# alexmillerdb/two_tower_recommender_model

Hardware: AMD Instinct MI355X
Metric: training pairs/sec at batch 8192 (per GPU) (higher is better)
Workload: dtype fp32; 1 GPU; northstar: 100M items x 50M users, emb_dim 128, towers [128, 64], single-hot uniform ids; global_batch=8192, per_gpu_batch=8192, emb_dim=128, tower_dtype=bf16 (MFMA, fp32 acc), parallelism=single-gpu hipgraph

## Files before the change

two_tower_recommender_model_amd/csrc/tower_rows.hip:

```cpp
#include "tower_common.h"

namespace tt {


constexpr int RK_THREADS = 320;
__device__ __forceinline__ int rk_perm(int mt, int rho) {
  return 32 * (mt >> 1) + 8 * (rho >> 2) + 4 * (mt & 1) + (rho & 3);
}
__device__ __forceinline__ bf16x8 rk_afwd(const char* img, int mt, int s, int rho, int q) {
  return *reinterpret_cast<const bf16x8*>(img + rk_off(rk_perm(mt, rho), 32 * s + 8 * q));
}
__device__ __forceinline__ bf16x8 rk_abwd(const char* img, int mt, int s, int lane) {
  const int q = lane >> 4, qq = (lane >> 2) & 3, p = lane & 3;
  const int row = 32 * s + 8 * q + qq;
  const int col = 32 * (mt >> 1) + 8 * p + 4 * (mt & 1);
  const bf16x4 lo = __builtin_amdgcn_ds_read_tr16_b64_v4bf16((lds_bf16x4*)(img + rk_off(row, col)));
  const bf16x4 hi = __builtin_amdgcn_ds_read_tr16_b64_v4bf16((lds_bf16x4*)(img + rk_off(row + 4, col)));
  return __builtin_shufflevector(lo, hi, 0, 1, 2, 3, 4, 5, 6, 7);
}
__device__ __forceinline__ bf16x8 rk_pack(const f32x4& a, const f32x4& b) {
  bf16x8 v;
#pragma unroll
  for (int j = 0; j < 4; ++j) {
    v[j] = (__bf16)a[j];
    v[4 + j] = (__bf16)b[j];
  }
  return v;
}
template <int MT, int S, bool BWD>
__device__ __forceinline__ void rk_gemm(f32x4 (&acc)[8], const char* img, const bf16x8 (&b)[4], int lane) {
  const int n = lane & 15, q = lane >> 4;
  bf16x8 fa[2][MT];
#pragma unroll
  for (int mt = 0; mt < MT; ++mt) {
    acc[mt] = (f32x4)(0.f);
    fa[0][mt] = BWD ? rk_abwd(img, mt, 0, lane) : rk_afwd(img, mt, 0, n, q);
  }
#pragma unroll
  for (int s = 0; s < S; ++s) {
    if (s + 1 < S) {
#pragma unroll
      for (int mt = 0; mt < MT; ++mt)
        fa[(s + 1) & 1][mt] = BWD ? rk_abwd(img, mt, s + 1, lane) : rk_afwd(img, mt, s + 1, n, q);
    }
    __builtin_amdgcn_sched_barrier(0);
#pragma unroll
    for (int mt = 0; mt < MT; ++mt)
      acc[mt] = __builtin_amdgcn_mfma_f32_16x16x32_bf16(fa[s & 1][mt], b[s], acc[mt], 0, 0, 0);
    __builtin_amdgcn_sched_barrier(0);
  }
}
template <int X>
__device__ __forceinline__ float rk_xor(float v) {
  if constexpr (X == 1) return dpp_f<0xB1>(v);
  if constexpr (X == 2) return dpp_f<0x4E>(v);
  if constexpr (X == 4) return dpp_f<0x1B>(dpp_f<0x141>(v));
  return dpp_f<0x128>(v);
}
template <int X, int H>
__device__ __forceinline__ void rk_halve(float* v, int n) {
  const bool up = (n & X) != 0;
#pragma unroll
  for (int i = 0; i < H; ++i) {
    const float keep = up ? v[H + i] : v[i], send = up ? v[i] : v[H + i];
    v[i] = keep + rk_xor<X>(send);
  }
}
template <int NV>
__device__ __forceinline__ void rk_colsum(float (&v)[NV], int n) {
  static_assert(NV == 32 || NV == 16, "column sum of 32 or 16 values per lane");
  rk_halve<8, NV / 2>(v, n);
  rk_halve<4, NV / 4>(v, n);
  rk_halve<2, NV / 8>(v, n);
  rk_halve<1, NV / 16>(v, n);
}
template <int NS>
__device__ __forceinline__ void rk_strip(const bf16x8 (&v)[4], __bf16* row, int q) {
#pragma unroll
  for (int s = 0; s < NS; ++s) *reinterpret_cast<bf16x8*>(row + 32 * s + 8 * q) = v[s];
}

__device__ __forceinline__ char* px_row(const tt_peer_direct_t& x, int64_t row, int64_t row_bytes) {
  char* base = reinterpret_cast<char*>(x.row0[0]);
  int64_t f0 = 0;
#pragma unroll
  for (int q = 1; q < TT_PEER_MAXW; ++q) {
    if (q < x.W && row >= x.first_row[q]) {
      base = reinterpret_cast<char*>(x.row0[q]);
      f0 = x.first_row[q];
    }
  }
  return base + (row - f0) * row_bytes;
}
__device__ __forceinline__ bool px_copy_unit(const tt_peer_direct_t& x, int64_t u, const uint4*& src, uint4*& dst) {
  int64_t pre = 0;
  bool hit = false;
#pragma unroll
  for (int q = 0; q < TT_PEER_MAXW; ++q) {
    const int64_t n = q < x.W ? x.copy_len[q] >> 4 : 0;
    if (!hit && u >= pre && u < pre + n) {
      src = reinterpret_cast<const uint4*>(x.copy_src[q]) + (u - pre);
      dst = reinterpret_cast<uint4*>(x.copy_dst[q]) + (u - pre);
      hit = true;
    }
    pre += n;
  }
  return hit;
}
__device__ __forceinline__ int64_t px_copy_units(const tt_peer_direct_t& x) {
  int64_t n = 0;
#pragma unroll
  for (int q = 0; q < TT_PEER_MAXW; ++q) n += q < x.W ? x.copy_len[q] >> 4 : 0;
  return n;
}

struct RkRaw {
  uint32_t lo, hi;
};
__device__ __forceinline__ RkRaw rk_raw(const void* p, bool wide, int64_t i) {
  RkRaw r;
  if (wide) {
    const uint2 v = reinterpret_cast<const uint2*>(p)[i];
    r.lo = v.x;
    r.hi = v.y;
  } else {
    r.lo = reinterpret_cast<const uint32_t*>(p)[i];
    r.hi = 0u;
  }
  return r;
}
__device__ __forceinline__ int64_t rk_id(RkRaw r, bool wide) {
  return wide ? (int64_t)(((uint64_t)r.hi << 32) | r.lo) : (int64_t)(int32_t)r.lo;
}
__device__ __forceinline__ float rk_label(RkRaw r, int dt) {
  if (dt == TT_I32) return (float)(int32_t)r.lo;
  if (dt == TT_I64) return (float)(int64_t)(((uint64_t)r.hi << 32) | r.lo);
  return __uint_as_float(r.lo);
}
template <int N, typename T>
__device__ __forceinline__ void rk_pin(T (&p)[N]) {
  static_assert(N == 2 || N == 4 || N == 8, "2, 4 or 8 values");
  if constexpr (N == 8)
    asm volatile("" : "+v"(p[0]), "+v"(p[1]), "+v"(p[2]), "+v"(p[3]), "+v"(p[4]), "+v"(p[5]), "+v"(p[6]), "+v"(p[7]));
  else if constexpr (N == 4)
    asm volatile("" : "+v"(p[0]), "+v"(p[1]), "+v"(p[2]), "+v"(p[3]));
  else
    asm volatile("" : "+v"(p[0]), "+v"(p[1]));
}
#if TT_EXPERIMENTS
#define RK_STAMP(k) \
  do { if (a.stamps && lane == 0) a.stamps[8192 + ((int64_t)blockIdx.x * 16 + (k)) * 9 + wid] = (int64_t)__builtin_amdgcn_s_memrealtime(); } while (0)
#define RK_STAMP2(k) \
  do { if (a.stamps && lane == 0) a.stamps[8192 + ((int64_t)blockIdx.x * 16 + (k)) * 9 + 4 + wid] = (int64_t)__builtin_amdgcn_s_memrealtime(); } while (0)
#define RK_STAMP_IMG(k) \
  do { if (a.stamps && lane == 0) a.stamps[8192 + ((int64_t)blockIdx.x * 16 + (k)) * 9 + 8] = (int64_t)__builtin_amdgcn_s_memrealtime(); } while (0)
#else
#define RK_STAMP(k) do { } while (0)
#define RK_STAMP2(k) do { } while (0)
#define RK_STAMP_IMG(k) do { } while (0)
#endif

template <bool UPD, bool IDX, int IN, bool POOL = false>
__device__ __forceinline__ void tower_rows_body(const TowerArgs& a) {
  static_assert(IN == 128 || IN == 64, "row-owned T1: inputs of 128 or 64");
  static_assert(!POOL || (!UPD && !IDX), "pooled input: the plain T1 only");
  constexpr int NI = IN / 32;
  constexpr int MTI = IN / 16;
  __shared__ __attribute__((aligned(16))) char wimg[RK_IMG];
  __shared__ __attribute__((aligned(16))) float xo[2][2][16 * 64];
  __shared__ float bsum[2][RK_W0 + RK_W1];
  __shared__ float lrow[TR];
  __shared__ __attribute__((aligned(16))) float xr[4][16 * IN];
  const int lane = threadIdx.x & 63, wid = __builtin_amdgcn_readfirstlane(threadIdx.x >> 6);
  typedef __attribute__((address_space(3))) void lds_void;
  typedef __attribute__((address_space(1))) void glb_void;
  if (wid == 4) {
    RK_STAMP_IMG(0);
    if (!TDBG(16)) {
#pragma unroll
      for (int k = 0; k < RK_IMG / 1024; ++k)
        __builtin_amdgcn_global_load_lds((glb_void*)(a.wimg + k * 1024 + lane * 16), (lds_void*)(wimg + k * 1024), 16, 0, 0);
    }
    RK_STAMP_IMG(1);
    __builtin_amdgcn_s_waitcnt(0x0F70);
    RK_STAMP_IMG(2);
    __syncthreads();
    RK_STAMP_IMG(3);
    __syncthreads();
    __syncthreads();
    return;
  }
  const int t = wid >> 1, h = wid & 1, q = lane >> 4, n = lane & 15;
  const RkCommon& C = a.rk.c;
  const RkTower& T = a.rk.tw[t];
  const int64_t B = C.B;
  const void* const labels = C.labels;
  const int label_dtype = C.label_dtype, gid_dtype = C.gid_dtype;
  const void* const idcol = T.idcol;
  const void* const tab0 = T.tab;
  const int64_t gmod = T.gmod;
  const float* const b0p = T.b0;
  const float* const b1p = T.b1;
  const int32_t* const claim = T.claim;
  const int32_t* const pos_out = T.pos_out;
  const int64_t pstride = T.rstride;
  const int nwg = C.nwg;
  if (UPD) asm volatile("" ::"s"(nwg), "s"(B), "s"(labels), "s"(label_dtype), "s"(gid_dtype), "s"(idcol), "s"(tab0), "s"(gmod), "s"(b0p), "s"(b1p), "s"(claim));
  else if (IDX) asm volatile("" ::"s"(nwg), "s"(B), "s"(labels), "s"(label_dtype), "s"(idcol), "s"(tab0), "s"(b0p), "s"(b1p), "s"(pos_out));
  else if (POOL) asm volatile("" ::"s"(nwg), "s"(B), "s"(labels), "s"(label_dtype), "s"(tab0), "s"(b0p), "s"(b1p), "s"(pstride));
  else asm volatile("" ::"s"(nwg), "s"(B), "s"(labels), "s"(label_dtype), "s"(gid_dtype), "s"(idcol), "s"(tab0), "s"(gmod), "s"(b0p), "s"(b1p));
  const int tile = xcd_remap((int)blockIdx.x, nwg);
  const int64_t m0 = (int64_t)tile * TR, m = m0 + 16 * h + n;
  const bool live = m < B;
  RK_STAMP(0);
  const bool wide = gid_dtype == TT_I64;
  const int64_t mc = live ? m : 0;
  RkRaw id_raw{0u, 0u}, pout_raw{0u, 0u};
  if (IDX) {
    id_raw.lo = (uint32_t) reinterpret_cast<const int32_t*>(idcol)[mc];
    pout_raw.lo = pos_out ? (uint32_t)pos_out[mc] : id_raw.lo;
  } else if (!POOL) {
    id_raw = rk_raw(idcol, wide, mc);
  }
  int32_t cl = -1;
  if (UPD) cl = claim[mc];
  const RkRaw lab_raw = rk_raw(labels, label_dtype == TT_I64, mc);
  f32x4 b0v[8], b1v[4];
  auto load_biases = [&]() {
#pragma unroll
    for (int mt = 0; mt < 8; ++mt) b0v[mt] = *reinterpret_cast<const f32x4*>(b0p + 32 * (mt >> 1) + 8 * q + 4 * (mt & 1));
#pragma unroll
    for (int mt = 0; mt < 4; ++mt) b1v[mt] = *reinterpret_cast<const f32x4*>(b1p + 32 * (mt >> 1) + 8 * q + 4 * (mt & 1));
  };
  load_biases();
  __builtin_amdgcn_sched_barrier(0);
  uint4 cpv = make_uint4(0u, 0u, 0u, 0u);
  uint4* cpd = nullptr;
  int64_t cp_per = 0, cp_end = 0;
  if constexpr (IDX) {
    if (a.xd.W) {
      const int64_t tot = px_copy_units(a.xd);
      cp_per = (tot + gridDim.x - 1) / gridDim.x;
      cp_end = min(tot, ((int64_t)blockIdx.x + 1) * cp_per);
      const int64_t u = (int64_t)blockIdx.x * cp_per + threadIdx.x;
      const uint4* cps;
      if (u < cp_end && px_copy_unit(a.xd, u, cps, cpd)) cpv = *cps;
      else cpd = nullptr;
    }
  }
  int64_t r;
  if (POOL) {
    r = live ? m : -1;
  } else if (IDX) {
    r = live ? (int64_t)(int32_t)id_raw.lo : -1;
  } else {
    const int64_t id = live ? rk_id(id_raw, wide) : 0;
    r = id != 0 ? py_mod64(id, gmod) : -1;
  }
  const float* tab = reinterpret_cast<const float*>(tab0);
  const int64_t rstride = POOL ? pstride : IN;
  RK_STAMP2(4);
  __builtin_amdgcn_sched_barrier(0);
  float* xw = xr[wid];
  constexpr int CPR = IDX ? IN / 8 : IN / 4;
  constexpr int RPI = 64 / CPR;
  constexpr int NDMA = 16 / RPI;
  if (IDX) {
    const int rr0 = lane / CPR, pc = lane % CPR;
    const char* src0 = reinterpret_cast<const char*>(tab0);
    const char* src[NDMA];
    int64_t rid[NDMA];
#pragma unroll
    for (int i = 0; i < NDMA; ++i) rid[i] = __shfl((long long)r, RPI * i + rr0, 64);
    rk_pin<NDMA>(rid);
#pragma unroll
    for (int i = 0; i < NDMA; ++i) {
      const int row = RPI * i + rr0;
      src[i] = src0 + (rid[i] >= 0 ? rid[i] : 0) * (IN * 2) + 16 * (pc ^ (row & (CPR - 1)));
    }
    rk_pin<NDMA>(src);
#pragma unroll
    for (int i = 0; i < NDMA; ++i)
      __builtin_amdgcn_global_load_lds((glb_void*)src[i], (lds_void*)(reinterpret_cast<char*>(xw) + i * 1024), 16, 0, 0);
  } else {
    const int rr0 = lane / CPR, pc = lane % CPR;
    const float* src[NDMA];
    int64_t rid[NDMA];
#pragma unroll
    for (int i = 0; i < NDMA; ++i) rid[i] = __shfl((long long)r, RPI * i + rr0, 64);
    rk_pin<NDMA>(rid);
#pragma unroll
    for (int i = 0; i < NDMA; ++i) {
      const int row = RPI * i + rr0;
      src[i] = tab + (rid[i] >= 0 ? rid[i] : 0) * rstride + 4 * (pc ^ row);
    }
    rk_pin<NDMA>(src);
#pragma unroll
    for (int i = 0; i < NDMA; ++i)
      if (!TDBG(32))
        __builtin_amdgcn_global_load_lds((glb_void*)src[i], (lds_void*)(xw + i * 256), 16, 0, 0);
  }
  __builtin_amdgcn_sched_barrier(0);
  DdPend pend;
  pend.key = DD_EMPTY;
  const int32_t li = (int32_t)(t * B + m);
  if (!UPD && a.dd_on && q == 0 && live) {
    const uint64_t key = r >= 0 ? (((uint64_t)(t ? a.dd_table[1] : a.dd_table[0]) << DD_TABLE_SHIFT) | (uint64_t)r)
                                : DD_EMPTY;
    dd_insert_begin(a.dd, key, li, pend);
  }
  RK_STAMP(1);
  const int in_max = C.in_max;
  const float grad_scale = C.grad_scale, fB = C.fB;
  DSlot* const slots = C.slots;
  __bf16* const xt_t = T.xt;
  __bf16* const act_t = T.act0;
  const float* const us_t = T.us;
  __builtin_amdgcn_sched_barrier(0);
  __builtin_amdgcn_s_waitcnt(0x0F70);
  if (UPD) asm volatile("" ::"s"(in_max), "s"(grad_scale), "s"(fB), "s"(slots), "s"(xt_t), "s"(act_t), "s"(us_t));
  else asm volatile("" ::"s"(in_max), "s"(grad_scale), "s"(fB), "s"(xt_t), "s"(act_t));
  RK_STAMP(2);
  __syncthreads();
  RK_STAMP(3);
  f32x4 xv[8];
  bf16x8 xb[4];
  if (IDX) {
#pragma unroll
    for (int s2 = 0; s2 < NI; ++s2) {
      const bf16x8 v = *reinterpret_cast<const bf16x8*>(reinterpret_cast<const char*>(xw) + n * (IN * 2) +
                                                         16 * ((4 * s2 + q) ^ (n & (CPR - 1))));
      xb[s2] = r >= 0 ? v : (bf16x8)(__bf16)0.f;
    }
  } else {
#pragma unroll
    for (int mt = 0; mt < MTI; ++mt) {
      const int c = 8 * (mt >> 1) + 2 * q + (mt & 1);
      const f32x4 v = *reinterpret_cast<const f32x4*>(xw + n * IN + 4 * (c ^ n));
      xv[mt] = r >= 0 ? v : (f32x4)(0.f);
    }
#pragma unroll
    for (int s2 = 0; s2 < NI; ++s2) xb[s2] = rk_pack(xv[2 * s2], xv[2 * s2 + 1]);
  }
  uint32_t word = 0u;
  float s_old = 0.f;
  if (UPD) {
    if (blockIdx.x == 0 && threadIdx.x == 0) {
      int32_t* const ctr = C.ctr;
      const int32_t nh = ctr[0];
      ctr[2] = nh;
      ctr[0] = 0;
    }
    word = reinterpret_cast<const uint32_t*>(&slots[cl >= 0 ? cl : 0].word)[0];
    s_old = us_t[r >= 0 ? r : 0];
  }
  __builtin_amdgcn_sched_barrier(0);
  const char* img0 = wimg + t * RK_IMG_T;
  const char* img1 = img0 + RK_W0 * 256;
  f32x4 acc[8];
  if (!TDBG(512)) rk_strip<NI>(xb, xt_t + m * in_max, q);
  rk_gemm<8, NI, false>(acc, img0, xb, lane);
  RK_STAMP(4);
  bf16x8 hb[4];
#pragma unroll
  for (int s = 0; s < 4; ++s) {
    f32x4 u0, u1;
#pragma unroll
    for (int j = 0; j < 4; ++j) {
      u0[j] = fmaxf(acc[2 * s][j] + b0v[2 * s][j], 0.f);
      u1[j] = fmaxf(acc[2 * s + 1][j] + b0v[2 * s + 1][j], 0.f);
    }
    hb[s] = rk_pack(u0, u1);
  }
  if (!TDBG(256)) rk_strip<4>(hb, act_t + m * MAXW, q);
  f32x4 uo[4];
  rk_gemm<4, 4, false>(acc, img1, hb, lane);
#pragma unroll
  for (int mt = 0; mt < 4; ++mt) uo[mt] = acc[mt];
#pragma unroll
  for (int mt = 0; mt < 4; ++mt) {
#pragma unroll
    for (int j = 0; j < 4; ++j) uo[mt][j] = fmaxf(uo[mt][j] + b1v[mt][j], 0.f);
    const int c = 8 * (mt >> 1) + 2 * q + (mt & 1);
    *reinterpret_cast<f32x4*>(&xo[t][h][n * 64 + ((c ^ n) << 2)]) = uo[mt];
  }
  RK_STAMP(5);
  RK_STAMP(6);
  __syncthreads();
  RK_STAMP(7);
  f32x4 vo[4];
#pragma unroll
  for (int mt = 0; mt < 4; ++mt) {
    const int c = 8 * (mt >> 1) + 2 * q + (mt & 1);
    vo[mt] = *reinterpret_cast<const f32x4*>(&xo[t ^ 1][h][n * 64 + ((c ^ n) << 2)]);
  }
  float gs[4];
#pragma unroll
  for (int mt = 0; mt < 4; ++mt) {
    float e = 0.f;
#pragma unroll
    for (int j = 0; j < 4; ++j) e = fmaf(uo[mt][j], vo[mt][j], e);
    gs[mt] = e;
  }
  float c0 = gs[0] + gs[1], c1 = gs[2] + gs[3];
  c0 += __shfl_xor(c0, 16, 64);
  c1 += __shfl_xor(c1, 16, 64);
  c0 += __shfl_xor(c0, 32, 64);
  c1 += __shfl_xor(c1, 32, 64);
  const float d = c0 + c1;
  float lo = 0.f, dl = 0.f;
  if (live) {
    const float x = d, y = rk_label(lab_raw, label_dtype);
    const float e = __expf(-fabsf(x));
    const float l1p = e < 1e-4f ? e * (1.f - 0.5f * e) : __logf(1.f + e);
    const float lsig = fminf(x, 0.f) - l1p;
    lo = (1.f - y) * x - lsig;
    const float rc = __builtin_amdgcn_rcpf(1.f + e);
    dl = ((x >= 0.f ? rc : e * rc) - y) * (grad_scale / fB);
  }
  const int hv = (int)(threadIdx.x >> 6) & 1;
  if (t == 0 && q == 0) lrow[16 * hv + n] = lo;
  float z1[16];
  bf16x8 z1b[4];
#pragma unroll
  for (int mt = 0; mt < 4; ++mt)
#pragma unroll
    for (int j = 0; j < 4; ++j) z1[4 * mt + j] = live && uo[mt][j] > 0.f ? dl * vo[mt][j] : 0.f;
#pragma unroll
  for (int s = 0; s < 2; ++s) {
    bf16x8 v;
#pragma unroll
    for (int j = 0; j < 8; ++j) v[j] = (__bf16)z1[8 * s + j];
    z1b[s] = v;
  }
  RK_STAMP(8);
  __bf16* const dzt0_t = T.dzt0;
  __bf16* const dzt1_t = T.dzt1;
  float* const uw_t = T.uw;
  const float ulr = C.ulr, ueps = C.ueps;
  int32_t* const multi = C.multi;
  const int nseg = C.nseg;
  rk_gemm<8, 2, true>(acc, img1, z1b, lane);
  if (UPD) asm volatile("" ::"s"(dzt0_t), "s"(dzt1_t), "s"(uw_t), "s"(ulr), "s"(ueps), "s"(multi), "s"(nseg));
  else asm volatile("" ::"s"(dzt0_t), "s"(dzt1_t));
  float z0[32];
  bf16x8 z0b[4];
#pragma unroll
  for (int mt = 0; mt < 8; ++mt)
#pragma unroll
    for (int j = 0; j < 4; ++j)
      z0[4 * mt + j] = live && (float)hb[mt >> 1][4 * (mt & 1) + j] > 0.f ? acc[mt][j] : 0.f;
#pragma unroll
  for (int s = 0; s < 4; ++s) {
    bf16x8 v;
#pragma unroll
    for (int j = 0; j < 8; ++j) v[j] = (__bf16)z0[8 * s + j];
    z0b[s] = v;
  }
  if (!TDBG(512)) rk_strip<2>(z1b, dzt1_t + m * MAXW, q);
  if (!TDBG(128)) rk_strip<4>(z0b, dzt0_t + m * MAXW, q);
  RK_STAMP(9);
  float* grow_t = nullptr;
  float* prow_t = nullptr;
  int64_t ldp = 0;
  float* db0_t = nullptr;
  float* db1_t = nullptr;
  float* logits = nullptr;
  float* loss_part = nullptr;
  if constexpr (!UPD) {
    grow_t = T.grow;
    prow_t = T.prow;
    ldp = C.ldp;
    db0_t = T.db0;
    db1_t = T.db1;
    logits = C.logits;
    loss_part = C.loss_part;
  }
  rk_gemm<MTI, 4, true>(acc, img0, z0b, lane);
  if constexpr (!UPD) asm volatile("" ::"s"(grow_t), "s"(prow_t), "s"(ldp), "s"(db0_t), "s"(db1_t), "s"(logits), "s"(loss_part));
  RK_STAMP(10);
  float* grow = nullptr;
  bool store_dx;
  if (IDX) {
    const int32_t po = (int32_t)pout_raw.lo;
    store_dx = r >= 0 && po >= 0;
    grow = grow_t + (int64_t)(store_dx ? po : 0) * IN;
    if (a.xd.W) grow = reinterpret_cast<float*>(px_row(a.xd, store_dx ? po : 0, IN * 4));
  } else {
    store_dx = live;
  }
  if (UPD) {
    float e2[2];
#pragma unroll
    for (int hh = 0; hh < 2; ++hh) {
      const float s0 = rw_sq4(acc[0 + hh]), s1 = rw_sq4(acc[2 + hh]);
      float c2;
      if constexpr (IN == 128) {
        const float s2 = rw_sq4(acc[4 + hh]), s3 = rw_sq4(acc[6 + hh]);
        c2 = (s0 + s2) + (s1 + s3);
      } else {
        c2 = s0 + s1;
      }
      c2 += __shfl_xor(c2, 32, 64);
      c2 += __shfl_xor(c2, 16, 64);
      e2[hh] = c2;
    }
    RK_STAMP2(0);
    const float sq = e2[0] + e2[1];
    const float snew = rw_state(s_old, sq, IN);
    const float step = rw_step(snew, ulr, ueps);
    const uint32_t cnt = word & (uint32_t)DD_CNT_MASK;
    const bool single = r >= 0 && cl >= 0 && cnt == 1u;
    {
      const bool mul = q == 0 && r >= 0 && cl >= 0 && cnt >= 2u && cnt <= (uint32_t)DD_INL;
      const uint64_t bal = __ballot(mul);
      const int seg = tile * 4 + wid;
      if (seg < nseg) {
        if (mul) multi[(int64_t)seg * DD_SEGW + 1 + __popcll(bal & ((1ull << lane) - 1))] = cl;
        if (lane == 0) multi[(int64_t)seg * DD_SEGW] = __popcll(bal);
      }
    }
#pragma unroll
    for (int mt = 0; mt < MTI; ++mt) {
      const int c = 8 * (mt >> 1) + 2 * q + (mt & 1);
      *reinterpret_cast<f32x4*>(xw + n * IN + 4 * (c ^ n)) = rw_apply(xv[mt], acc[mt], step);
    }
    RK_STAMP2(1);
    asm volatile("" ::: "memory");
    {
      const int rr0 = lane / CPR, pc = lane % CPR;
      float* wtab = uw_t;
      const int64_t rsend = single ? r : -1;
      int64_t rid[NDMA];
      f32x4 w[NDMA];
      grow_t = T.grow;
      prow_t = T.prow;
      ldp = C.ldp;
      db0_t = T.db0;
      db1_t = T.db1;
      logits = C.logits;
      loss_part = C.loss_part;
#pragma unroll
      for (int i = 0; i < NDMA; ++i) rid[i] = __shfl((long long)rsend, RPI * i + rr0, 64);
#pragma unroll
      for (int i = 0; i < NDMA; ++i) w[i] = *reinterpret_cast<const f32x4*>(xw + (RPI * i + rr0) * IN + 4 * pc);
      rk_pin<NDMA>(rid);
      rk_pin<NDMA>(w);
      asm volatile("" ::"s"(grow_t), "s"(prow_t), "s"(ldp), "s"(db0_t), "s"(db1_t), "s"(logits), "s"(loss_part));
#pragma unroll
      for (int i = 0; i < NDMA; ++i) {
        const int row = RPI * i + rr0;
        if (__builtin_expect(rid[i] >= 0, 1)) *reinterpret_cast<f32x4*>(wtab + rid[i] * IN + 4 * (pc ^ row)) = w[i];
      }
    }
    RK_STAMP2(2);
    if (single) {
      if (q == 0) {
        const_cast<float*>(us_t)[r] = snew;
        slots[cl].word = DD_EMPTY;
      }
      store_dx = prow_t != nullptr;
    }
  }
  if (!IDX) grow = grow_t + m * ldp;
  if (store_dx) {
#pragma unroll
    for (int mt = 0; mt < MTI; ++mt)
      *reinterpret_cast<f32x4*>(grow + 32 * (mt >> 1) + 8 * q + 4 * (mt & 1)) = acc[mt];
  }
  RK_STAMP2(3);
  if (t == 0 && q == 0 && live) logits[m] = d;
  if (!IDX && !POOL && prow_t && live) {
    float* prow = prow_t + m * ldp;
#pragma unroll
    for (int mt = 0; mt < MTI; ++mt) *reinterpret_cast<f32x4*>(prow + 32 * (mt >> 1) + 8 * q + 4 * (mt & 1)) = xv[mt];
  }
  RK_STAMP(11);
  RK_STAMP(12);
  rk_colsum<32>(z0, n);
  rk_colsum<16>(z1, n);
  auto feat = [&](int k) { return 32 * ((k >> 2) >> 1) + 8 * q + 4 * ((k >> 2) & 1) + (k & 3); };
  if (hv == 1) {
    bsum[t][feat(2 * n)] = z0[0];
    bsum[t][feat(2 * n + 1)] = z0[1];
    bsum[t][RK_W0 + feat(n)] = z1[0];
  }
  RK_STAMP(13);
  __syncthreads();
  RK_STAMP(14);
  if (hv == 0) {
    float* db0 = db0_t + (int64_t)tile * MAXW;
    float* db1 = db1_t + (int64_t)tile * MAXW;
    db0[feat(2 * n)] = z0[0] + bsum[t][feat(2 * n)];
    db0[feat(2 * n + 1)] = z0[1] + bsum[t][feat(2 * n + 1)];
    db1[feat(n)] = z1[0] + bsum[t][RK_W0 + feat(n)];
    if (t == 0 && lane == 0) {
      float p = 0.f;
      for (int i = 0; i < TR; ++i) p += lrow[i];
      loss_part[tile] = p;
    }
  }
  if (!UPD && a.dd_on && q == 0) dd_insert_defer_finish_at(a.dd, pend, li, tile, 16 * wid + n);
  if constexpr (IDX) {
    if (cpd) *cpd = cpv;
    if (a.xd.W) {
      for (int64_t u = (int64_t)blockIdx.x * cp_per + threadIdx.x + 256; u < cp_end; u += 256) {
        const uint4* s2;
        uint4* d2;
        if (px_copy_unit(a.xd, u, s2, d2)) *d2 = *s2;
      }
    }
    if (a.xd.epoch && blockIdx.x == 0 && threadIdx.x == 0)
      __hip_atomic_fetch_add(a.xd.epoch, 1, __ATOMIC_RELAXED, __HIP_MEMORY_SCOPE_AGENT);
  }
  RK_STAMP(15);
}
template <bool UPD, bool IDX = false, int IN = 128, bool POOL = false>
__global__ void __launch_bounds__(RK_THREADS) tower_rows_kernel(TowerArgs a) {
  tower_rows_body<UPD, IDX, IN, POOL>(a);
}

static void rk_front(TowerArgs& a, bool pool) {
  RkCommon& c = a.rk.c;
  c.B = a.B;
  c.labels = a.labels;
  c.label_dtype = a.label_dtype;
  c.gid_dtype = a.gid_dtype;
  c.grad_scale = a.grad_scale;
  c.in_max = (int32_t)a.in_max;
  c.slots = a.dd.slots;
  c.ctr = a.dd.ctr;
  c.ulr = a.ulr;
  c.nwg = a.nwg;
  c.fB = (float)a.B;
  c.ueps = a.ueps;
  c.ldp = a.ldp;
  c.multi = a.dd.multi;
  c.logits = a.logits;
  c.loss_part = a.loss_part;
  c.nseg = a.dd.nseg;
  const bool idx = a.gpos[0] != nullptr;
  for (int t = 0; t < 2; ++t) {
    RkTower& w = a.rk.tw[t];
    w.idcol = idx ? static_cast<const void*>(a.gpos[t]) : a.gcol[t];
    w.tab = idx ? static_cast<const void*>(a.gsrc[t]) : pool ? static_cast<const void*>(a.pooled + a.s.in_col[t]) : a.gtab[t];
    w.gmod = a.gmod[t];
    w.b0 = a.params + a.boff[t][0];
    w.b1 = a.params + a.boff[t][1];
    w.claim = a.uw[0] ? a.dd.claim + (int64_t)t * a.B : nullptr;
    w.pos_out = a.gpos_out[0] ? a.gpos_out[t] : nullptr;
    w.rstride = a.ldp;
    w.xt = a.xt + (int64_t)t * a.in_max * a.Bp;
    w.act0 = a.act + ((int64_t)t * MAXL + 0) * MAXW * a.Bp;
    w.dzt0 = a.dzt + ((int64_t)t * MAXL + 0) * MAXW * a.Bp;
    w.dzt1 = a.dzt + ((int64_t)t * MAXL + 1) * MAXW * a.Bp;
    w.us = a.us[t];
    w.uw = a.uw[t];
    w.grow = idx ? a.gdst[t] : a.gpooled + a.s.in_col[t];
    w.prow = a.pooled_out ? a.pooled_out + a.s.in_col[t] : nullptr;
    w.db0 = a.dbpart + ((int64_t)t * MAXL + 0) * a.nwg * MAXW;
    w.db1 = a.dbpart + ((int64_t)t * MAXL + 1) * a.nwg * MAXW;
  }
}

int launch_t1_rows(TowerArgs& a, void* stream) {
  const dim3 g(a.nwg), b(RK_THREADS);
  const bool in64 = a.s.in_dim[0] == 64;
  if (!a.gcol[0] && !a.gpos[0]) {
    rk_front(a, true);
    in64 ? tower_rows_kernel<false, false, 64, true><<<g, b, 0, as_stream(stream)>>>(a)
         : tower_rows_kernel<false, false, 128, true><<<g, b, 0, as_stream(stream)>>>(a);
    return check_launch("tower_rows_pooled");
  }
  rk_front(a, false);
  if (a.gpos[0])
    in64 ? tower_rows_kernel<false, true, 64><<<g, b, 0, as_stream(stream)>>>(a)
         : tower_rows_kernel<false, true, 128><<<g, b, 0, as_stream(stream)>>>(a);
  else if (a.uw[0])
    in64 ? tower_rows_kernel<true, false, 64><<<g, b, 0, as_stream(stream)>>>(a)
         : tower_rows_kernel<true, false, 128><<<g, b, 0, as_stream(stream)>>>(a);
  else
    in64 ? tower_rows_kernel<false, false, 64><<<g, b, 0, as_stream(stream)>>>(a)
         : tower_rows_kernel<false, false, 128><<<g, b, 0, as_stream(stream)>>>(a);
  return check_launch(a.uw[0] ? "tower_rows_gather_update" : "tower_rows_gather");
}

}
```

Before: 298.1 million pairs/s.

## Chain GEMM fragment prefetch across products and interleave column sums with MFMAs

The row-owned tower kernel now keeps one double-buffered A-fragment set shared across the four chained GEMMs. During the last k-step of each product it prefetches the next product's first fragments, so LDS latency at each GEMM boundary is hidden. The bias-gradient column reductions (DPP halving) are split into levels and issued between the MFMAs of the backward GEMMs instead of running serially afterwards. Scalar argument loads are moved to overlap barriers, the xt strip store is placed after the first fragment load, and the loss partial is read as vector LDS loads. The risk is higher register pressure from the shared fragment buffers and tighter scheduling constraints.

```diff
diff --git a/two_tower_recommender_model_amd/csrc/tower_rows.hip b/two_tower_recommender_model_amd/csrc/tower_rows.hip
--- a/two_tower_recommender_model_amd/csrc/tower_rows.hip
+++ b/two_tower_recommender_model_amd/csrc/tower_rows.hip
@@ -27,23 +27,24 @@
   }
   return v;
 }
-template <int MT, int S, bool BWD>
-__device__ __forceinline__ void rk_gemm(f32x4 (&acc)[8], const char* img, const bf16x8 (&b)[4], int lane) {
+template <int MT, bool BWD>
+__device__ __forceinline__ void rk_frags(bf16x8 (&f)[8], const char* img, int s, int lane) {
   const int n = lane & 15, q = lane >> 4;
-  bf16x8 fa[2][MT];
-#pragma unroll
-  for (int mt = 0; mt < MT; ++mt) {
-    acc[mt] = (f32x4)(0.f);
-    fa[0][mt] = BWD ? rk_abwd(img, mt, 0, lane) : rk_afwd(img, mt, 0, n, q);
-  }
+#pragma unroll
+  for (int mt = 0; mt < MT; ++mt) f[mt] = BWD ? rk_abwd(img, mt, s, lane) : rk_afwd(img, mt, s, n, q);
+}
+template <int MT, int S, bool BWD, typename Next, typename Fill>
+__device__ __forceinline__ void rk_gemm(f32x4 (&acc)[8], bf16x8 (&fa)[2][8], const char* img, const bf16x8 (&b)[4],
+                                        int lane, Next next, Fill fill) {
+  static_assert(S % 2 == 0, "the next product's k-step 0 goes to set 0");
+#pragma unroll
+  for (int mt = 0; mt < MT; ++mt) acc[mt] = (f32x4)(0.f);
 #pragma unroll
   for (int s = 0; s < S; ++s) {
-    if (s + 1 < S) {
-#pragma unroll
-      for (int mt = 0; mt < MT; ++mt)
-        fa[(s + 1) & 1][mt] = BWD ? rk_abwd(img, mt, s + 1, lane) : rk_afwd(img, mt, s + 1, n, q);
-    }
+    if (s + 1 < S) rk_frags<MT, BWD>(fa[(s + 1) & 1], img, s + 1, lane);
+    else next(fa[(s + 1) & 1]);
     __builtin_amdgcn_sched_barrier(0);
+    fill(s);
 #pragma unroll
     for (int mt = 0; mt < MT; ++mt)
       acc[mt] = __builtin_amdgcn_mfma_f32_16x16x32_bf16(fa[s & 1][mt], b[s], acc[mt], 0, 0, 0);
@@ -67,12 +68,12 @@
   }
 }
 template <int NV>
-__device__ __forceinline__ void rk_colsum(float (&v)[NV], int n) {
+__device__ __forceinline__ void rk_colsum_level(float (&v)[NV], int n, int l) {
   static_assert(NV == 32 || NV == 16, "column sum of 32 or 16 values per lane");
-  rk_halve<8, NV / 2>(v, n);
-  rk_halve<4, NV / 4>(v, n);
-  rk_halve<2, NV / 8>(v, n);
-  rk_halve<1, NV / 16>(v, n);
+  if (l == 0) rk_halve<8, NV / 2>(v, n);
+  else if (l == 1) rk_halve<4, NV / 4>(v, n);
+  else if (l == 2) rk_halve<2, NV / 8>(v, n);
+  else rk_halve<1, NV / 16>(v, n);
 }
 template <int NS>
 __device__ __forceinline__ void rk_strip(const bf16x8 (&v)[4], __bf16* row, int q) {
@@ -169,7 +170,7 @@
   __shared__ __attribute__((aligned(16))) char wimg[RK_IMG];
   __shared__ __attribute__((aligned(16))) float xo[2][2][16 * 64];
   __shared__ float bsum[2][RK_W0 + RK_W1];
-  __shared__ float lrow[TR];
+  __shared__ __attribute__((aligned(16))) float lrow[TR];
   __shared__ __attribute__((aligned(16))) float xr[4][16 * IN];
   const int lane = threadIdx.x & 63, wid = __builtin_amdgcn_readfirstlane(threadIdx.x >> 6);
   typedef __attribute__((address_space(3))) void lds_void;
@@ -321,8 +322,6 @@
   if (UPD) asm volatile("" ::"s"(in_max), "s"(grad_scale), "s"(fB), "s"(slots), "s"(xt_t), "s"(act_t), "s"(us_t));
   else asm volatile("" ::"s"(in_max), "s"(grad_scale), "s"(fB), "s"(xt_t), "s"(act_t));
   RK_STAMP(2);
-  __syncthreads();
-  RK_STAMP(3);
   f32x4 xv[8];
   bf16x8 xb[4];
   if (IDX) {
@@ -341,6 +340,21 @@
     }
 #pragma unroll
     for (int s2 = 0; s2 < NI; ++s2) xb[s2] = rk_pack(xv[2 * s2], xv[2 * s2 + 1]);
+  }
+  typedef __attribute__((address_space(1))) bf16x8 glb_bf16x8;
+  glb_bf16x8* xrow = (glb_bf16x8*)(xt_t + m * in_max);
+  asm volatile("" : "+v"(xrow));
+  __builtin_amdgcn_sched_barrier(0);
+  __syncthreads();
+  RK_STAMP(3);
+  const char* img0 = wimg + t * RK_IMG_T;
+  const char* img1 = img0 + RK_W0 * 256;
+  bf16x8 fa[2][8];
+  rk_frags<8, false>(fa[0], img0, 0, lane);
+  __builtin_amdgcn_sched_barrier(0);
+  if (!TDBG(512)) {
+#pragma unroll
+    for (int s = 0; s < NI; ++s) xrow[4 * s + q] = xb[s];
   }
   uint32_t word = 0u;
   float s_old = 0.f;
@@ -355,11 +369,9 @@
     s_old = us_t[r >= 0 ? r : 0];
   }
   __builtin_amdgcn_sched_barrier(0);
-  const char* img0 = wimg + t * RK_IMG_T;
-  const char* img1 = img0 + RK_W0 * 256;
+  auto no_fill = [](int) {};
   f32x4 acc[8];
-  if (!TDBG(512)) rk_strip<NI>(xb, xt_t + m * in_max, q);
-  rk_gemm<8, NI, false>(acc, img0, xb, lane);
+  rk_gemm<8, NI, false>(acc, fa, img0, xb, lane, [&](bf16x8(&f)[8]) { rk_frags<4, false>(f, img1, 0, lane); }, no_fill);
   RK_STAMP(4);
   bf16x8 hb[4];
 #pragma unroll
@@ -374,7 +386,23 @@
   }
   if (!TDBG(256)) rk_strip<4>(hb, act_t + m * MAXW, q);
   f32x4 uo[4];
-  rk_gemm<4, 4, false>(acc, img1, hb, lane);
+  rk_gemm<4, 4, false>(acc, fa, img1, hb, lane, [&](bf16x8(&f)[8]) { rk_frags<8, true>(f, img1, 0, lane); }, no_fill);
+  __bf16* const dzt0_t = T.dzt0;
+  __bf16* const dzt1_t = T.dzt1;
+  float* const uw_t = T.uw;
+  const float ulr = C.ulr, ueps = C.ueps;
+  const int nseg = C.nseg;
+  float* grow_t = nullptr;
+  float* prow_t = nullptr;
+  int64_t ldp = 0;
+  float* logits = nullptr;
+  if constexpr (!UPD) {
+    grow_t = T.grow;
+    prow_t = T.prow;
+    ldp = C.ldp;
+    logits = C.logits;
+  }
+  __builtin_amdgcn_sched_barrier(0);
 #pragma unroll
   for (int mt = 0; mt < 4; ++mt) uo[mt] = acc[mt];
 #pragma unroll
@@ -387,6 +415,8 @@
   RK_STAMP(5);
   RK_STAMP(6);
   __syncthreads();
+  if (UPD) asm volatile("" ::"s"(dzt0_t), "s"(dzt1_t), "s"(uw_t), "s"(ulr), "s"(ueps), "s"(nseg));
+  else asm volatile("" ::"s"(dzt0_t), "s"(dzt1_t), "s"(grow_t), "s"(prow_t), "s"(ldp), "s"(logits));
   RK_STAMP(7);
   f32x4 vo[4];
 #pragma unroll
@@ -418,8 +448,13 @@
     const float rc = __builtin_amdgcn_rcpf(1.f + e);
     dl = ((x >= 0.f ? rc : e * rc) - y) * (grad_scale / fB);
   }
-  const int hv = (int)(threadIdx.x >> 6) & 1;
-  if (t == 0 && q == 0) lrow[16 * hv + n] = lo;
+  auto tid = [] {
+    uint32_t v = threadIdx.x;
+    asm volatile("" : "+v"(v));
+    return v;
+  };
+  const int hv = (int)(tid() >> 6) & 1;
+  if ((tid() & 0xB0u) == 0u) lrow[16 * hv + n] = lo;
   float z1[16];
   bf16x8 z1b[4];
 #pragma unroll
@@ -434,15 +469,11 @@
     z1b[s] = v;
   }
   RK_STAMP(8);
-  __bf16* const dzt0_t = T.dzt0;
-  __bf16* const dzt1_t = T.dzt1;
-  float* const uw_t = T.uw;
-  const float ulr = C.ulr, ueps = C.ueps;
-  int32_t* const multi = C.multi;
-  const int nseg = C.nseg;
-  rk_gemm<8, 2, true>(acc, img1, z1b, lane);
-  if (UPD) asm volatile("" ::"s"(dzt0_t), "s"(dzt1_t), "s"(uw_t), "s"(ulr), "s"(ueps), "s"(multi), "s"(nseg));
-  else asm volatile("" ::"s"(dzt0_t), "s"(dzt1_t));
+  rk_gemm<8, 2, true>(acc, fa, img1, z1b, lane, [&](bf16x8(&f)[8]) { rk_frags<MTI, true>(f, img0, 0, lane); },
+                      [&](int s) {
+                        rk_colsum_level<16>(z1, n, 2 * s);
+                        rk_colsum_level<16>(z1, n, 2 * s + 1);
+                      });
   float z0[32];
   bf16x8 z0b[4];
 #pragma unroll
@@ -460,24 +491,14 @@
   if (!TDBG(512)) rk_strip<2>(z1b, dzt1_t + m * MAXW, q);
   if (!TDBG(128)) rk_strip<4>(z0b, dzt0_t + m * MAXW, q);
   RK_STAMP(9);
-  float* grow_t = nullptr;
-  float* prow_t = nullptr;
-  int64_t ldp = 0;
-  float* db0_t = nullptr;
-  float* db1_t = nullptr;
-  float* logits = nullptr;
-  float* loss_part = nullptr;
-  if constexpr (!UPD) {
-    grow_t = T.grow;
-    prow_t = T.prow;
-    ldp = C.ldp;
-    db0_t = T.db0;
-    db1_t = T.db1;
-    logits = C.logits;
-    loss_part = C.loss_part;
-  }
-  rk_gemm<MTI, 4, true>(acc, img0, z0b, lane);
-  if constexpr (!UPD) asm volatile("" ::"s"(grow_t), "s"(prow_t), "s"(ldp), "s"(db0_t), "s"(db1_t), "s"(logits), "s"(loss_part));
+  rk_gemm<MTI, 4, true>(acc, fa, img0, z0b, lane, [](bf16x8(&)[8]) {},
+                        [&](int s) { rk_colsum_level<32>(z0, n, s); });
+  auto feat = [&](int k) { return 32 * ((k >> 2) >> 1) + 8 * q + 4 * ((k >> 2) & 1) + (k & 3); };
+  if (hv == 1) {
+    bsum[t][feat(2 * n)] = z0[0];
+    bsum[t][feat(2 * n + 1)] = z0[1];
+    bsum[t][RK_W0 + feat(n)] = z1[0];
+  }
   RK_STAMP(10);
   float* grow = nullptr;
   bool store_dx;
@@ -490,6 +511,8 @@
     store_dx = live;
   }
   if (UPD) {
+    int32_t* const multi = C.multi;
+    __builtin_amdgcn_sched_barrier(0);
     float e2[2];
 #pragma unroll
     for (int hh = 0; hh < 2; ++hh) {
@@ -505,10 +528,12 @@
       c2 += __shfl_xor(c2, 16, 64);
       e2[hh] = c2;
     }
+    asm volatile("" ::"s"(multi));
     RK_STAMP2(0);
     const float sq = e2[0] + e2[1];
     const float snew = rw_state(s_old, sq, IN);
     const float step = rw_step(snew, ulr, ueps);
+    float* us_w;
     const uint32_t cnt = word & (uint32_t)DD_CNT_MASK;
     const bool single = r >= 0 && cl >= 0 && cnt == 1u;
     {
@@ -528,7 +553,8 @@
     RK_STAMP2(1);
     asm volatile("" ::: "memory");
     {
-      const int rr0 = lane / CPR, pc = lane % CPR;
+      const int wl = (int)(tid() & 63u);
+      const int rr0 = wl / CPR, pc = wl % CPR;
       float* wtab = uw_t;
       const int64_t rsend = single ? r : -1;
       int64_t rid[NDMA];
@@ -536,17 +562,17 @@
       grow_t = T.grow;
       prow_t = T.prow;
       ldp = C.ldp;
-      db0_t = T.db0;
-      db1_t = T.db1;
       logits = C.logits;
-      loss_part = C.loss_part;
+      int tw = t;
+      asm volatile("" : "+s"(tw));
+      us_w = const_cast<float*>(a.rk.tw[tw].us);
 #pragma unroll
       for (int i = 0; i < NDMA; ++i) rid[i] = __shfl((long long)rsend, RPI * i + rr0, 64);
 #pragma unroll
       for (int i = 0; i < NDMA; ++i) w[i] = *reinterpret_cast<const f32x4*>(xw + (RPI * i + rr0) * IN + 4 * pc);
       rk_pin<NDMA>(rid);
       rk_pin<NDMA>(w);
-      asm volatile("" ::"s"(grow_t), "s"(prow_t), "s"(ldp), "s"(db0_t), "s"(db1_t), "s"(logits), "s"(loss_part));
+      asm volatile("" ::"s"(grow_t), "s"(prow_t), "s"(ldp), "s"(logits), "s"(us_w));
 #pragma unroll
       for (int i = 0; i < NDMA; ++i) {
         const int row = RPI * i + rr0;
@@ -556,7 +582,7 @@
     RK_STAMP2(2);
     if (single) {
       if (q == 0) {
-        const_cast<float*>(us_t)[r] = snew;
+        us_w[r] = snew;
         slots[cl].word = DD_EMPTY;
       }
       store_dx = prow_t != nullptr;
@@ -569,7 +595,7 @@
       *reinterpret_cast<f32x4*>(grow + 32 * (mt >> 1) + 8 * q + 4 * (mt & 1)) = acc[mt];
   }
   RK_STAMP2(3);
-  if (t == 0 && q == 0 && live) logits[m] = d;
+  if ((tid() & 0xB0u) == 0u && live) logits[m] = d;
   if (!IDX && !POOL && prow_t && live) {
     float* prow = prow_t + m * ldp;
 #pragma unroll
@@ -577,16 +603,13 @@
   }
   RK_STAMP(11);
   RK_STAMP(12);
-  rk_colsum<32>(z0, n);
-  rk_colsum<16>(z1, n);
-  auto feat = [&](int k) { return 32 * ((k >> 2) >> 1) + 8 * q + 4 * ((k >> 2) & 1) + (k & 3); };
-  if (hv == 1) {
-    bsum[t][feat(2 * n)] = z0[0];
-    bsum[t][feat(2 * n + 1)] = z0[1];
-    bsum[t][RK_W0 + feat(n)] = z1[0];
-  }
+  float* const db0_t = T.db0;
+  float* const db1_t = T.db1;
+  float* const loss_part = C.loss_part;
+  __builtin_amdgcn_sched_barrier(0);
   RK_STAMP(13);
   __syncthreads();
+  asm volatile("" ::"s"(db0_t), "s"(db1_t), "s"(loss_part));
   RK_STAMP(14);
   if (hv == 0) {
     float* db0 = db0_t + (int64_t)tile * MAXW;
@@ -594,9 +617,14 @@
     db0[feat(2 * n)] = z0[0] + bsum[t][feat(2 * n)];
     db0[feat(2 * n + 1)] = z0[1] + bsum[t][feat(2 * n + 1)];
     db1[feat(n)] = z1[0] + bsum[t][RK_W0 + feat(n)];
-    if (t == 0 && lane == 0) {
+    if (tid() == 0u) {
+      f32x4 lv[TR / 4];
+#pragma unroll
+      for (int i = 0; i < TR / 4; ++i) lv[i] = reinterpret_cast<const f32x4*>(lrow)[i];
+      rk_pin<TR / 4>(lv);
       float p = 0.f;
-      for (int i = 0; i < TR; ++i) p += lrow[i];
+#pragma unroll
+      for (int i = 0; i < TR; ++i) p += lv[i >> 2][i & 3];
       loss_part[tile] = p;
     }
   }
```

Result: faster. 303.8 million pairs/s (median of 6 runs) (+1.9%).
